# facebookresearch/Active-3D-Vision-and-Touch

Measured on AMD Instinct MI355X. Metric: mesh-recon iters/sec (fwd+bwd, 2562-vert GCN + 10k-pt Chamfer) at bs=64, higher is better.
Workload: dtype f32; 1 GPU; icosphere-4 template (2562 verts, 5120 faces), 3-stage GCN 20x300 cut 0.33, bs=64/GPU, 10000-pt Chamfer x3 draws, Adam, ellipsoid clouds (BASELINE.json configs[1]); global_batch=64, parallelism=dp1

## Files before the change

### active-3d-vision-and-touch_amd/csrc/capi.hip

```cpp
#include <stdarg.h>
#include <stdlib.h>
#include <string.h>

#include "../../include/a3vt.h"
#include <atomic>
#include <mutex>
#include <unordered_map>

#include "kernels.h"
#include "prims.h"

namespace a3vt {

static thread_local char g_err[512] = "";

void set_error(const char *fmt, ...) {
  va_list ap;
  va_start(ap, fmt);
  vsnprintf(g_err, sizeof(g_err), fmt, ap);
  va_end(ap);
}

__device__ float g_zero_page[64];
static const float *zero_page() {
// ... 178 lines not shown
  StackPlan p{};
  const size_t m = (size_t)batch * n_vert;
  p.x3 = mode == GEMM_FP32X3 && num_layers > 2 && rowgemm3_stack_ok((long long)m, hidden, mask_ld(hidden, cut_len));
  p.omode = mode == GEMM_BF16_OPERANDS ? GEMM_BF16_OPERANDS : GEMM_FP32;
  const bool split_ok = split_usable(split, n_vert, cut_len);
  p.quad = num_layers > 1 &&
           (rec >= 0 ? rec == 1 : use_csrq(batch, n_vert, hidden, cut_len, mode, split_ok ? csrq_max_degree() : max_degree));
  p.qsplit = p.quad && split_ok;
  p.qcols = p.quad ? kQuadCols : 0;
  p.rm_ld = hidden - p.qcols;
  p.rm_off = m * p.qcols;
  return p;
}

static int launch_stack_ell(const StackPlan &p, const a3vt_adj_split *split, const int32_t *rowptr, const int32_t *col,
                            const float *val, int n_vert, int32_t *ell, hipStream_t s) {
  if (p.qsplit) {
    const SplitRef r = split_ref(split);
    return launch_csrqs_image(r.rowptr, r.col, r.scale, r.cls, n_vert, ell, s);
  }
  return p.quad ? launch_csrq_ell(rowptr, col, val, n_vert, ell, s) : 0;
}

static StackLayout stack_layout(int batch, int n_vert, int in_features, int hidden, int num_layers, int cut_len,
                                int need_backward, int gemm_mode = 0) {
  StackLayout L{};
  const size_t m = (size_t)batch * n_vert;
  const int cpad = pad4(cut_len);
  Arena a;
  const int kmax = hidden > pad4(in_features) ? hidden : pad4(in_features);
  L.wt_stride = align_up((size_t)rowgemm_bt_rows(kmax) * pad16(kmax), 64);
  if (gemm_mode == GEMM_FP32X3 && L.wt_stride < 3 * (size_t)kX3ImageFloats) L.wt_stride = 3 * (size_t)kX3ImageFloats;
  L.wt = a.take(L.wt_stride * (num_layers > 1 ? num_layers - 1 : 1));
  L.ldza = cpad > 4 ? cpad : 4;
  L.za = a.take(m * L.ldza);
  L.z3 = a.take(2 * m * 4);
// ... 510 lines not shown
  if (int rc = hub_rows(rowptr, n_vert, max_degree, scratch + L.heavy, &heavy, s)) return rc;
  const StackPlan P = stack_plan(gemm_bf16, batch, n_vert, hidden, num_layers, cut_len, max_degree, split, -1);
  const int qcols = P.qcols, rm_ld = P.rm_ld;
  const size_t rm_off = P.rm_off;
  if (P.x3)
    if (int rc = launch_stack_images(GEMM_FP32X3, 1, weights, 1, num_layers - 1, in_features, hidden, ld_feats, hidden,
                                     scratch + L.wt, L.wt_stride, s))
      return rc;
  if (int rc = launch_stack_images(GEMM_FP32, 1, weights, 0, P.x3 ? 1 : num_layers - 1, in_features, hidden, ld_feats, hidden,
                                   scratch + L.wt, L.wt_stride, s))
    return rc;
  if (num_layers > 1) path_count(P.quad ? PATH_STACK_QUAD : PATH_STACK_ROWS);
  if (P.qsplit) path_count(PATH_STACK_SPLIT);
  if (num_layers > 1) stash_layout_record(masks, P.quad);
  int32_t *ell = reinterpret_cast<int32_t *>(scratch + L.ell);
  if (int rc = launch_stack_ell(P, split, rowptr, col, val, n_vert, ell, s)) return rc;
  const float *x = feats, *xq = nullptr;
  int ldx = ld_feats;
  for (int i = 0; i + 1 < num_layers; ++i) {
    const int k = i == 0 ? ld_feats : hidden;
    const bool l3 = P.x3 && i > 0;
    float *y = acts ? acts + S.act(i) : scratch + L.ping[i & 1];
    RowGemmArgs g{};
    g.a0 = g.a1 = x;
    g.lda0 = g.lda1 = ldx;
    g.ksplit = k;
    if (xq) {
      g.a0 = xq;
      g.ksplit = qcols;
      g.a0q_nvert = n_vert;
      g.a0q_quads = qcols / 4;
// ... 18 lines not shown
      g.zq_nvert = n_vert;
      g.zq_quads = cpad / 4;
      g.yq = y;
      g.yq_quads = qcols / 4;
      g.trash = scratch + L.z3;
    }
    {
      ProfScope ps(PROF_GEMM_FWD, s);
      if (int rc = launch_rowgemm(g, EPI_FWD_HIDDEN, s)) return rc;
    }
    if (P.quad) {
      uint8_t *sq = masks ? masks + S.signq(i) : nullptr;
      ProfScope psa(PROF_AGG, s);
      if (P.qsplit) {
        if (int rc = launch_csrqs_fwd(scratch + L.za, biases[i], cut_len, ell, n_vert, batch, y, qcols / 4, sq, 1, s)) return rc;
      } else if (int rc = launch_csrq_fwd(scratch + L.za, biases[i], cut_len, rowptr, col, val, heavy, ell, n_vert, batch, y, qcols / 4, sq, 1, s)) {
        return rc;
      }
      xq = y;
    } else if (cut_len > 0) {
      ProfScope psa(PROF_AGG, s);
      if (int rc = launch_csr_fwd(scratch + L.za, L.ldza, biases[i], cut_len, rowptr, col, val, heavy, n_vert, batch, y, hidden, mk, S.mld, 1, s))
        return rc;
    }
    x = y + rm_off - qcols;
    ldx = rm_ld;
  }
  const int klast = num_layers == 1 ? in_features : hidden;
  ProfScope pso(PROF_OUT, s);
  const SplitRef sref = split_ref(split);
  return launch_thin_fwd(x, ldx, klast, weights[num_layers - 1], biases[num_layers - 1], rowptr, col, val, heavy, n_vert,
// ... 50 lines not shown
  const StackLayout L = stack_layout(batch, n_vert, in_features, hidden, num_layers, cut_len, 1, gemm_bf16);
  const StackStash S = stack_stash(batch, n_vert, hidden, num_layers, cut_len, gemm_bf16);
  const size_t m = (size_t)batch * n_vert;
  const int cpad = pad4(cut_len);
  const int last = num_layers - 1;

  const SplitRef sref = split_ref(split);
  int32_t *heavyT;
  if (int rc = hub_rows(rowptrT, n_vert, max_degreeT, scratch + L.heavy, &heavyT, s)) return rc;
  const StackPlan P = stack_plan(gemm_bf16, batch, n_vert, hidden, num_layers, cut_len, max_degreeT, split,
                                 masks ? stash_layout_lookup(masks) : 0);
  const bool quad = P.quad;
  const int qcols = P.qcols, rm_ld = P.rm_ld;
  const size_t rm_off = P.rm_off;
  int32_t *ellT = reinterpret_cast<int32_t *>(scratch + L.ell);
  if (int rc = launch_stack_ell(P, split, rowptrT, colT, valT, n_vert, ellT, s)) return rc;
  {
    const float *xl = num_layers == 1 ? feats : acts + S.act(last - 1);
    const float *x = xl + rm_off - qcols;
    const int ldx = num_layers == 1 ? ld_feats : rm_ld;
    const int k = num_layers == 1 ? in_features : hidden;
    float *gprev = num_layers == 1 ? grad_feats : scratch + L.ping[0];
    const int ldg = num_layers == 1 ? ld_feats : hidden;
    ProfScope pso(PROF_OUT, s);
    if (int rc = launch_thin_bwd(x, ldx, k, weights[last], rowptrT, colT, valT, heavyT, n_vert, batch, grad_update,
                                 scratch + L.z3, num_layers > 1, gprev, ldg, ldg, scratch + L.thin_dw_slab,
                                 scratch + L.thin_db_slab, quad ? scratch + L.gq : nullptr, cpad / 4, quad ? xl : nullptr,
                                 qcols / 4, s, split ? &sref : nullptr))
      return rc;
    if (int rc = reduce_output_grads(scratch + L.thin_dw_slab, scratch + L.thin_db_slab, k, grad_weights[last], grad_biases[last],
                                     acc, s))
// ... 14 lines not shown
    float *g = scratch + L.ping[cur];
    float *dza = scratch + L.za;
    const float *xl = i == 0 ? feats : acts + S.act(i - 1);
    const bool xhyb = quad && i > 0;
    const float *x = xhyb ? xl + rm_off - qcols : xl;
    const int ldx = i == 0 ? ld_feats : (xhyb ? rm_ld : hidden);
    const int kin = i == 0 ? in_features : hidden;

    if (cut_len > 0 && quad) {
      const uint8_t *sq = masks + S.signq(i);
      ProfScope psa(PROF_AGG, s);
      if (P.qsplit) {
        if (int rc = launch_csrqs_bwd(scratch + L.gq, cut_len, ellT, n_vert, batch, dza, sq,
                                      scratch + L.db_slab + (size_t)i * L.db_layer_stride, s))
          return rc;
      } else if (int rc = launch_csrq_bwd(scratch + L.gq, cut_len, rowptrT, colT, valT, heavyT, ellT, n_vert, batch, dza, sq,
                                          scratch + L.db_slab + (size_t)i * L.db_layer_stride, s)) {
        return rc;
      }
    } else if (cut_len > 0) {
      ProfScope psa(PROF_AGG, s);
      if (int rc = launch_csr_bwd(g, hidden, cut_len, rowptrT, colT, valT, heavyT, n_vert, batch, dza, L.ldza,
                                  scratch + L.db_slab + (size_t)i * L.db_layer_stride, s))
        return rc;
    } else if (!acc) {
      if (int rc = launch_fill_zero(grad_biases[i], hidden, s)) return rc;
    }

    DwArgs d{};
    if (xhyb) {
      d.ldx_src = rm_ld;
// ... 809 lines not shown

int a3vt_dbg_path_counts(long long *counts, int n, int reset) {
  A3VT_CHECK_ARG(n >= 0 && (counts != nullptr || n == 0));
  for (int i = 0; i < n; ++i) counts[i] = i < PATH_COUNT ? g_path_counts[i].load(std::memory_order_relaxed) : 0;
  if (reset)
    for (auto &c : g_path_counts) c.store(0, std::memory_order_relaxed);
  return PATH_COUNT;
}

int a3vt_dbg_csr_algo(int algo) {
  A3VT_CHECK_ARG(algo >= 0 && algo <= 2);
  g_csr_algo = algo;
  return 0;
}

int a3vt_split3_bf16(const float *x, size_t n, uint16_t *hi, uint16_t *mid, uint16_t *lo, void *stream) {
  A3VT_CHECK_ARG(n == 0 || (x && hi && mid && lo));
  return launch_split3(x, n, hi, mid, lo, static_cast<hipStream_t>(stream));
}

int a3vt_check_finite(const float *data, size_t n, int32_t *flag, void *stream) {
  A3VT_CHECK_ARG(data && flag);
  return launch_check_finite(data, n, flag, static_cast<hipStream_t>(stream));
}

}
```

### active-3d-vision-and-touch_amd/csrc/gcn_csrq.hip

```cpp
#include "kernels.h"
#include "prims.h"

namespace a3vt {


constexpr int kCsrqThreads = 512;
constexpr int kHeavyDegQ = 64;
constexpr int kEllW = 8;

__global__ void csr_ell_build_kernel(const int32_t *__restrict__ rowptr, const int32_t *__restrict__ colidx,
                                     const float *__restrict__ val, int n_vert, i32x2 *__restrict__ ell,
                                     int32_t *__restrict__ degs) {
  const int v = blockIdx.x * blockDim.x + threadIdx.x;
  if (v >= n_vert) return;
  const int e0 = rowptr[v], n = rowptr[v + 1] - e0;
  degs[v] = n;
#pragma unroll
  for (int j = 0; j < kEllW; ++j)
    ell[(size_t)j * n_vert + v] = j < n ? i32x2{colidx[e0 + j], (int)f32_bits(val[e0 + j])} : i32x2{n_vert, 0};
}
size_t csrq_ell_ints(int n_vert) { return (size_t)n_vert * (2 * kEllW + 1) + 64; }
int launch_csrq_ell(const int32_t *rowptr, const int32_t *col, const float *val, int n_vert, int32_t *ell, hipStream_t s) {
  A3VT_LAUNCH(csr_ell_build_kernel, dim3(cdiv(n_vert, 256)), dim3(256), 0, s, rowptr, col, val, n_vert,
              reinterpret_cast<i32x2 *>(ell), ell + (size_t)n_vert * 2 * kEllW);
  A3VT_CHECK_LAUNCH();
  return 0;
}

template <int MODE, int VPT>
__global__ __launch_bounds__(kCsrqThreads) void csrq_kernel(const float *__restrict__ srcq, int nq, int parts,
                                                            const float *__restrict__ bias, int c,
                                                            const int32_t *__restrict__ rowptr,
                                                            const int32_t *__restrict__ colidx,
                                                            const float *__restrict__ val, int n_vert, int batch,
                                                            float *__restrict__ dst, int nq_dst,
                                                            uint8_t *__restrict__ signq, int relu, int heavy_thresh,
                                                            float *__restrict__ db_slab,
                                                            const int32_t *__restrict__ ellbuf) {
  extern __shared__ __attribute__((aligned(16))) float lds_raw[];
  __shared__ float red[2][kCsrqThreads / 64][4];
  const i32x2 *ell = reinterpret_cast<const i32x2 *>(ellbuf);
  const int32_t *degs = ellbuf + (size_t)n_vert * 2 * kEllW;
  f32x4 *tile0 = reinterpret_cast<f32x4 *>(lds_raw);
  const int xcd = blockIdx.x & 7, loc = blockIdx.x >> 3;
  const int jm = loc / parts, part = loc - jm * parts;
  const int b = xcd + 8 * jm;
  if (b >= batch) return;
  const int q_lo = part * nq / parts, q_hi = (part + 1) * nq / parts;
  if (q_lo >= q_hi) return;

  int vv[VPT], dg[VPT];
  bool on[VPT];
  int cj[VPT][kEllW];
  float wj[VPT][kEllW];
#pragma unroll
  for (int k = 0; k < VPT; ++k) {
    const int v = threadIdx.x + k * kCsrqThreads;
    on[k] = v < n_vert;
    vv[k] = on[k] ? v : n_vert - 1;
    dg[k] = degs[vv[k]];
#pragma unroll
    for (int j = 0; j < kEllW; ++j) {
      const i32x2 e = ell[(size_t)j * n_vert + vv[k]];
      const int e0 = e[0], e1 = e[1];
      cj[k][j] = e0;
      wj[k][j] = bits_f32((unsigned)e1);
    }
  }

  auto fetch = [&](int q, int k, f32x4 &v4, unsigned &bits) {
    const size_t plane = ((size_t)b * nq + q) * n_vert;
    v4 = reinterpret_cast<const f32x4 *>(srcq)[plane + vv[k]];
    bits = MODE == 1 ? signq[plane + vv[k]] : 0u;
  };
  auto park = [&](f32x4 *tile, int q, int k, f32x4 v4, unsigned bits) {
    if (MODE == 1) {
#pragma unroll
      for (int t = 0; t < 4; ++t) v4[t] = ((bits >> t) & 1u) ? v4[t] : 0.f;
    }
    (void)q;
    tile[vv[k]] = v4;
  };

  if (threadIdx.x < 2) tile0[(size_t)threadIdx.x * (n_vert + 1) + n_vert] = f32x4{0.f, 0.f, 0.f, 0.f};
  {
    f32x4 v4[VPT];
    unsigned bits[VPT];
#pragma unroll
    for (int k = 0; k < VPT; ++k) fetch(q_lo, k, v4[k], bits[k]);
#pragma unroll
    for (int k = 0; k < VPT; ++k) park(tile0, q_lo, k, v4[k], bits[k]);
  }
  __syncthreads();

  for (int q = q_lo; q < q_hi; ++q) {
    const int par = (q - q_lo) & 1;
    const f32x4 *tile = tile0 + (size_t)par * (n_vert + 1);
    f32x4 *tnext = tile0 + (size_t)(par ^ 1) * (n_vert + 1);
    const int ch = q * 4;
    const size_t plane = ((size_t)b * nq + q) * n_vert;
    const int qn = q + 1 < q_hi ? q + 1 : q;
    f32x4 nv4[VPT];
    unsigned nbits[VPT];
#pragma unroll
    for (int k = 0; k < VPT; ++k) fetch(qn, k, nv4[k], nbits[k]);
    f32x4 bs = {0.f, 0.f, 0.f, 0.f};
    if (MODE == 0) {
#pragma unroll
      for (int t = 0; t < 4; ++t)
        if (ch + t < c) bs[t] = bias[ch + t];
    }
    f32x4 bsum = {0.f, 0.f, 0.f, 0.f};
#pragma unroll
    for (int k = 0; k < VPT; ++k) {
      __builtin_amdgcn_sched_barrier(0);
      const int v = vv[k];
      const f32x4 own = tile[v];
      if (MODE == 1) {
#pragma unroll
        for (int t = 0; t < 4; ++t) bsum[t] += on[k] ? own[t] : 0.f;
      }
      f32x4 acc = {0.f, 0.f, 0.f, 0.f};
#pragma unroll
      for (int j = 0; j < kEllW; ++j) {
        {
          const f32x4 r = tile[cj[k][j]];
          const float w = wj[k][j];
          acc[0] = __builtin_fmaf(w, r[0], acc[0]);
          acc[1] = __builtin_fmaf(w, r[1], acc[1]);
          acc[2] = __builtin_fmaf(w, r[2], acc[2]);
          acc[3] = __builtin_fmaf(w, r[3], acc[3]);
        }
      }
      if (dg[k] > kEllW && dg[k] <= heavy_thresh) {
        const int ea = rowptr[v];
        for (int e = ea + kEllW; e < ea + dg[k]; ++e) {
          const f32x4 r = tile[colidx[e]];
          const float w = val[e];
#pragma unroll
          for (int t = 0; t < 4; ++t) acc[t] = __builtin_fmaf(w, r[t], acc[t]);
        }
      }
      if (!on[k] || dg[k] > heavy_thresh) continue;
      f32x4 o;
      if (MODE == 0) {
        unsigned bits = 0;
#pragma unroll
        for (int t = 0; t < 4; ++t) {
          const float pre = ch + t < c ? acc[t] + bs[t] : own[t];
          o[t] = (pre > 0.f || !relu) ? pre : 0.f;
          bits |= (pre > 0.f ? 1u : 0u) << t;
// ... 2 lines not shown
      } else {
#pragma unroll
        for (int t = 0; t < 4; ++t) o[t] = ch + t < c ? acc[t] : own[t];
      }
      *reinterpret_cast<f32x4 *>(dst + ((((size_t)b * nq_dst + q) * n_vert) + v) * 4) = o;
    }
    __builtin_amdgcn_sched_barrier(0);
    if (MODE == 1) {
#pragma unroll
      for (int t = 0; t < 4; ++t) bsum[t] = wave_sum(bsum[t]);
      if ((threadIdx.x & 63) == 0) {
#pragma unroll
        for (int t = 0; t < 4; ++t) red[par][threadIdx.x >> 6][t] = bsum[t];
      }
    }
    if (q + 1 < q_hi) {
#pragma unroll
      for (int k = 0; k < VPT; ++k) park(tnext, q + 1, k, nv4[k], nbits[k]);
    }
    __syncthreads();
    if (MODE == 1 && threadIdx.x < 4) {
      float sacc = 0.f;
#pragma unroll
      for (int w = 0; w < kCsrqThreads / 64; ++w) sacc += red[par][w][threadIdx.x];
      db_slab[(size_t)b * (nq * 4) + ch + threadIdx.x] = sacc;
    }
  }
}

template <int MODE>
__global__ __launch_bounds__(256) void csrq_heavy_kernel(const float *__restrict__ srcq, int nq,
                                                         const float *__restrict__ bias, int c,
                                                         const int32_t *__restrict__ rowptr,
                                                         const int32_t *__restrict__ colidx,
                                                         const float *__restrict__ val, int n_vert, int batch,
                                                         const int32_t *__restrict__ heavy, float *__restrict__ dst,
                                                         int nq_dst, uint8_t *__restrict__ signq, int relu) {
  __shared__ f32x4 red[8][32];
  const int hl = threadIdx.x & 31, sub = threadIdx.x >> 5;
  const int count = heavy[0];
  const bool on = hl < nq;
// ... 41 lines not shown
        const unsigned bits = signq[plane + v];
#pragma unroll
        for (int t = 0; t < 4; ++t) {
          own[t] = ((bits >> t) & 1u) ? own[t] : 0.f;
          o[t] = ch + t < c ? a[t] : own[t];
        }
      }
      *reinterpret_cast<f32x4 *>(dst + ((((size_t)b * nq_dst + hl) * n_vert) + v) * 4) = o;
    }
    __syncthreads();
  }
}

int csrq_max_degree() { return kEllW; }
bool csrq_fits(int n_vert, int cut_len) {
  return cut_len > 0 && pad4(cut_len) <= 128 && n_vert <= 6 * kCsrqThreads && ((size_t)n_vert + 1) * 32 <= 158 * 1024;
}

template <int MODE, int VPT>
static int launch_csrq_vpt(const float *srcq, int nq, const float *bias, int c, const int32_t *rowptr, const int32_t *col,
                           const float *val, const int32_t *heavy, const int32_t *ell, int n_vert, int batch, float *dst,
                           int nq_dst, uint8_t *signq, int relu, float *db_slab, hipStream_t s) {
  const size_t shmem = ((size_t)n_vert + 1) * 32;
  static OncePerDevice once;
  once.run([] {
    (void)hipFuncSetAttribute((const void *)csrq_kernel<MODE, VPT>, hipFuncAttributeMaxDynamicSharedMemorySize, 158 * 1024);
  });
  int parts = 256 / (((batch + 7) / 8) * 8);
  parts = parts < 1 ? 1 : parts > nq ? nq : parts;
  const int grid = 8 * ((batch + 7) / 8) * parts;
  A3VT_LAUNCH((csrq_kernel<MODE, VPT>), dim3(grid), dim3(kCsrqThreads), shmem, s, srcq, nq, parts, bias, c, rowptr, col, val,
              n_vert, batch, dst, nq_dst, signq, relu, heavy ? kHeavyDegQ : 0x7fffffff, db_slab, ell);
  A3VT_CHECK_LAUNCH();
  return 0;
}

template <int MODE>
static int launch_csrq(const float *srcq, const float *bias, int c, const int32_t *rowptr, const int32_t *col,
                       const float *val, const int32_t *heavy, const int32_t *ell, int n_vert, int batch, float *dst,
                       int nq_dst, uint8_t *signq, int relu, float *db_slab, hipStream_t s) {
  const int nq = pad4(c) / 4;
  if (!csrq_fits(n_vert, c) || nq_dst < nq || (MODE == 1 && (!signq || !db_slab))) {
    set_error("csrq: n_vert=%d c=%d output planes=%d unsupported", n_vert, c, nq_dst);
    return -1;
  }
  int rc;
  if (n_vert <= 4 * kCsrqThreads)
    rc = launch_csrq_vpt<MODE, 4>(srcq, nq, bias, c, rowptr, col, val, heavy, ell, n_vert, batch, dst, nq_dst, signq, relu, db_slab, s);
  else
    rc = launch_csrq_vpt<MODE, 6>(srcq, nq, bias, c, rowptr, col, val, heavy, ell, n_vert, batch, dst, nq_dst, signq, relu, db_slab, s);
  if (rc) return rc;
  if (heavy) {
    A3VT_LAUNCH(csrq_heavy_kernel<MODE>, dim3(2048), dim3(256), 0, s, srcq, nq, bias, c, rowptr, col, val, n_vert, batch,
                heavy, dst, nq_dst, signq, relu);
    A3VT_CHECK_LAUNCH();
  }
  return 0;
}

int launch_csrq_fwd(const float *zq, const float *bias, int c, const int32_t *rowptr, const int32_t *col,
                    const float *val, const int32_t *heavy, const int32_t *ell, int n_vert, int batch, float *yq,
                    int yq_quads, uint8_t *signq, int relu, hipStream_t s) {
  return launch_csrq<0>(zq, bias, c, rowptr, col, val, heavy, ell, n_vert, batch, yq, yq_quads, signq, relu, nullptr, s);
}
int launch_csrq_bwd(const float *gq, int c, const int32_t *rowptrT, const int32_t *colT, const float *valT,
                    const int32_t *heavyT, const int32_t *ellT, int n_vert, int batch, float *dzaq,
                    const uint8_t *signq, float *db_slab, hipStream_t s) {
  return launch_csrq<1>(gq, nullptr, c, rowptrT, colT, valT, heavyT, ellT, n_vert, batch, dzaq, pad4(c) / 4,
                        const_cast<uint8_t *>(signq), 0, db_slab, s);
}

}
```

### active-3d-vision-and-touch_amd/csrc/kernels.h

```cpp
#pragma once
#include <hip/hip_runtime.h>
#include <stddef.h>
#include <stdint.h>

namespace a3vt {

enum { EPI_PLAIN = 0, EPI_FWD_HIDDEN = 1, EPI_DX_MASK = 2 };
enum GemmMode { GEMM_FP32 = 0, GEMM_BF16_OPERANDS = 1, GEMM_BF16_STORAGE = 2, GEMM_FP32X3 = 3 };

struct RowGemmArgs {
  const float *a0;
  const float *a1;
  const float *bt;
  const float *zeros;
  uint8_t *maskb;
  float *c;
  float *c2;
  int lda0, lda1, ksplit, ldb;
  int bt_rows;
  int col0;
  int m, k, n_store;
  int ldc, ldc2, csplit, mld, moff;
  int no_relu;
  int plain_relu;
// ... 71 lines not shown

int launch_csr_fwd(const float *za, int ldza, const float *bias, int c, const int32_t *rowptr, const int32_t *col,
                   const float *val, const int32_t *heavy, int n_vert, int batch, float *y, int ldy, uint8_t *maskb,
                   int mld, int relu, hipStream_t s);
size_t csr_heavy_scratch_ints(int n_vert);
int csr_heavy_degree();
int launch_csr_heavy_list(const int32_t *rowptr, int n_vert, int32_t *heavy, hipStream_t s);
int launch_relu_split(const float *gy, int ldgy, const float *y, int ldy, int relu, int n_out, int cpad, int npad,
                      long long m, float *ga, float *dz, hipStream_t s);
int csr_bwd_num_slabs(int batch, int n_vert);
int launch_csr_bwd(const float *g, int ldg, int c, const int32_t *rowptrT, const int32_t *colT, const float *valT,
                   const int32_t *heavyT, int n_vert, int batch, float *dza, int lddza, float *db_slab, hipStream_t s);

bool csrq_fits(int n_vert, int cut_len);
int csrq_max_degree();
size_t csrq_ell_ints(int n_vert);
int launch_csrq_ell(const int32_t *rowptr, const int32_t *col, const float *val, int n_vert, int32_t *ell, hipStream_t s);
int launch_csrq_fwd(const float *zq, const float *bias, int c, const int32_t *rowptr, const int32_t *col,
                    const float *val, const int32_t *heavy, const int32_t *ell, int n_vert, int batch, float *yq,
                    int yq_quads ,
                    uint8_t *signq, int relu, hipStream_t s);
int launch_csrq_bwd(const float *gq, int c, const int32_t *rowptrT, const int32_t *colT, const float *valT,
                    const int32_t *heavyT, const int32_t *ellT, int n_vert, int batch, float *dzaq, const uint8_t *signq,
                    float *db_slab, hipStream_t s);
struct SplitRef {
  const int32_t *rowptr, *col;
  const float *scale;
  const uint8_t *cls;
};
bool csrqs_fits(int n_vert, int cut_len);
int csrqs_max_degree();
int launch_csrqs_image(const int32_t *rowptr, const int32_t *col, const float *scale, const uint8_t *cls, int n_vert,
                       int32_t *img, hipStream_t s);
int launch_csrqs_fwd(const float *zq, const float *bias, int c, const int32_t *img, int n_vert, int batch, float *yq,
                     int yq_quads, uint8_t *signq, int relu, hipStream_t s);
int launch_csrqs_bwd(const float *gq, int c, const int32_t *img, int n_vert, int batch, float *dzaq, const uint8_t *signq,
                     float *db_slab, hipStream_t s);
bool rowgemm_quad_major_ok(int m, int n_store, int cpad);

// ... 194 lines not shown
```

### active-3d-vision-and-touch_amd/lib.py

```python
import ctypes
import os
import subprocess

_HERE = os.path.dirname(os.path.abspath(__file__))
CSRC = os.path.join(_HERE, "csrc")
LIB_PATH = os.environ.get("A3VT_LIB", os.path.join(_HERE, "liba3vt.so"))
SOURCES = ["capi.hip", "gcn_gemm.hip", "gcn_gemmw.hip", "gcn_dww.hip", "gcn_gemm16.hip", "gcn_gemm3.hip", "gcn_csr.hip", "gcn_csrq.hip", "gcn_csrqs.hip", "gcn_bf16s.hip", "posenc.hip", "posenc_wide.hip", "bias_grad.hip", "bnrelu.hip", "conv5.hip", "conv5f.hip", "adam.hip", "sample.hip", "chamfer.hip", "nn_prune.hip",
           "pooling.hip", "fold.hip", "ddqn.hip", "qnet_input.hip", "latent_nn.hip"]
EXTRA_FLAGS = {"chamfer.hip": ["-fno-slp-vectorize"], "nn_prune.hip": ["-fno-slp-vectorize"],
               "gcn_csrq.hip": ["-fno-slp-vectorize"], "gcn_csrqs.hip": ["-fno-slp-vectorize"],
               "gcn_gemmw.hip": ["-std=c++20"], "gcn_dww.hip": ["-std=c++20"]}

_vp, _i, _sz, _u64 = ctypes.c_void_p, ctypes.c_int, ctypes.c_size_t, ctypes.c_uint64


class AdjSplit(ctypes.Structure):
    _fields_ = [("rowptr", _vp), ("col", _vp), ("scale", _vp), ("cls", _vp),
                ("max_degree", ctypes.c_int32), ("n_seam", ctypes.c_int32), ("n_centre", ctypes.c_int32)]


SIGNATURES = {
    "a3vt_version": (_i, []),
    "a3vt_last_error": (ctypes.c_char_p, []),
    "a3vt_csr_validate": (_i, [_vp, _vp, _i, _i]),
# ... 67 lines not shown
    "a3vt_fold_fwd": (_i, [_vp, _vp, _i, _vp, _vp, _vp, _vp, _vp, _i, _i, _i, _vp, _vp, _sz, _vp]),
    "a3vt_fold_bwd": (_i, [_vp, _vp, _i, _vp, _vp, _vp, _vp, _vp, _i, _i, _i, _vp, _vp, _vp, _vp, _vp, _vp, _vp, _vp, _sz, _vp]),
    "a3vt_ddqn_td": (_i, [_vp, _vp, _vp, _vp, _vp, _vp, _vp, _i, _i, _i, ctypes.c_float, _vp, _vp, _vp, _vp, _vp]),
    "a3vt_ddqn_td_bwd": (_i, [_vp, _vp, _vp, _i, _i, _vp, _vp]),
    "a3vt_latent_nearest_scratch_bytes": (_sz, [_i, _i, _i]),
    "a3vt_latent_nearest": (_i, [_vp, _vp, _i, _i, _vp, _vp, _i, _i, _i, _vp, _vp, _vp, _vp, _vp, _vp]),
    "a3vt_latent_nn_tile": (_i, []),
    "a3vt_latent_nn_query_floats": (_i, []),
    "a3vt_latent_nn_cached_rows": (_i, []),
    "a3vt_qnet_input_scratch_bytes": (_sz, [_i, _i, _i, _i, _i]),
    "a3vt_qnet_input_fwd": (_i, [_vp, _vp, _vp, _vp, _vp, _vp, _vp, _vp, _vp, _i, _i, _vp, _vp, _vp, _i, _i, _i, _vp, _i, _vp, _vp]),
    "a3vt_qnet_input_bwd": (_i, [_vp, _vp, _vp, _vp, _vp, _vp, _i, _i, _vp, _vp, _vp, _i, _i, _i, _vp, _i, _vp, _i,
                                 _vp, _vp, _vp, _vp, _vp, _vp, _vp, _vp, _vp, _vp]),
    "a3vt_dbg_csr_algo": (_i, [_i]),
    "a3vt_dbg_path_counts": (_i, [_vp, _i, _i]),
    "a3vt_dbg_nn_work": (_i, [_i, _vp]),
    "a3vt_split3_bf16": (_i, [_vp, _sz, _vp, _vp, _vp, _vp]),
    "a3vt_check_finite": (_i, [_vp, _sz, _vp, _vp]),
    "a3vt_profile_enable": (_i, [_i]),
    "a3vt_profile_read": (_i, [_vp, _vp]),
    "a3vt_profile_read_classes": (_i, [_vp, _vp, _i]),
}

_LIB = None


def build(force=False, verbose=False):
    return _build(force, verbose, LIB_PATH, os.path.join(_HERE, "build"))


# ... 58 lines not shown
```

### include/a3vt.h

```cpp
#ifndef A3VT_H
#define A3VT_H
#include <stddef.h>
#include <stdint.h>

#ifdef __cplusplus
extern "C" {
#endif

#define A3VT_VERSION 163

int a3vt_version(void);
const char *a3vt_last_error(void);

int a3vt_csr_validate(const int32_t *rowptr_host, const int32_t *col_host, int n_vert, int nnz);

size_t a3vt_gcn_stack_scratch_bytes(int batch, int n_vert, int in_features, int hidden, int num_layers,
                                    int cut_len, int need_backward);
size_t a3vt_gcn_stack_mask_bytes(int batch, int n_vert, int hidden, int num_layers, int cut_len);
size_t a3vt_gcn_stack_scratch_bytes_mode(int batch, int n_vert, int in_features, int hidden, int num_layers,
                                         int cut_len, int need_backward, int gemm_bf16);
int a3vt_gcn_stack_stash_bytes(int batch, int n_vert, int hidden, int num_layers, int cut_len, int gemm_bf16,
                               size_t *acts_bytes, size_t *mask_bytes);

int a3vt_gcn_stack_fwd(const float *feats, int ld_feats, int in_features,
// ... 159 lines not shown
                     float *dist_xy, int32_t *idx_xy, float *dist_yx, int32_t *idx_yx, float *cd,
                     void *scratch, void *stream);
size_t a3vt_chamfer_workspace_bytes(int draws, int batch, int p, int q);
int a3vt_chamfer_fwd_ws(const float *x, const float *y, int draws, int batch, int p, int q,
                        float *dist_xy, int32_t *idx_xy, float *dist_yx, int32_t *idx_yx, float *cd,
                        void *workspace, size_t workspace_bytes, int algo, void *stream);
int a3vt_chamfer_fwd_shared(const float *x, const float *y, int draws, int batch, int y_batch, int p, int q,
                            float *dist_xy, int32_t *idx_xy, float *dist_yx, int32_t *idx_yx, float *cd,
                            void *workspace, size_t workspace_bytes, int algo, void *stream);
int a3vt_chamfer_bwd(const float *x, const float *y, int draws, int batch, int p, int q,
                     const int32_t *idx_xy, const int32_t *idx_yx, const float *grad_cd,
                     float *grad_x, float *grad_y, void *stream);

int a3vt_dbg_csr_algo(int algo);

int a3vt_dbg_path_counts(long long *counts, int n, int reset);

int a3vt_dbg_nn_work(int enable, unsigned long long *out8);

int a3vt_split3_bf16(const float *x, size_t n, uint16_t *hi, uint16_t *mid, uint16_t *lo, void *stream);

size_t a3vt_fold_workspace_bytes(int batch, int points, int backward);
int a3vt_fold_fwd(const float *bias_s, const float *g, int k, const float *w1g, const float *w2, const float *b2, const float *w3,
                  const float *b3, int batch, int points, int width, float *y, void *workspace, size_t workspace_bytes, void *stream);
int a3vt_fold_bwd(const float *bias_s, const float *g, int k, const float *w1g, const float *w2, const float *b2, const float *w3,
                  const float *dy, int batch, int points, int width, float *d_bias_s, float *dg, float *dw1g, float *dw2, float *db2,
                  float *dw3, float *db3, void *workspace, size_t workspace_bytes, void *stream);

int a3vt_ddqn_td(const float *q_cur, const float *q_next_online, const float *q_next_target, const float *mask, const float *actions,
                 const float *rewards, const float *denom, int batch, int num_actions, int budget, float gamma, float *loss,
// ... 33 lines not shown
```

Before: 21.84 iters/s.

## Compact CSRQ ELL image, triple-buffer quad planes, and balance leftover quads

The ELL index image is rebuilt with separate weight and packed 16-bit byte-offset column planes, and its width is sized to the actual max degree (6–8). The CSRQ aggregation kernel now keeps a three-slot LDS ring with inline-asm loads and explicit vmcnt waits, so the next two quad planes are prefetched while the current one is gathered. Leftover quads that do not divide evenly across parts are split by vertex groups among all parts. This aims to cut register pressure and index traffic and to hide global load latency. In exchange it uses 1.5x more LDS per block, depends on hand-written waitcnt bookkeeping, and restricts n_vert so byte offsets fit in 16 bits.

```diff
diff --git a/active-3d-vision-and-touch_amd/csrc/capi.hip b/active-3d-vision-and-touch_amd/csrc/capi.hip
--- a/active-3d-vision-and-touch_amd/csrc/capi.hip
+++ b/active-3d-vision-and-touch_amd/csrc/capi.hip
@@ -216,12 +216,12 @@
 }
 
 static int launch_stack_ell(const StackPlan &p, const a3vt_adj_split *split, const int32_t *rowptr, const int32_t *col,
-                            const float *val, int n_vert, int32_t *ell, hipStream_t s) {
+                            const float *val, int n_vert, int slots, int32_t *ell, hipStream_t s) {
   if (p.qsplit) {
     const SplitRef r = split_ref(split);
     return launch_csrqs_image(r.rowptr, r.col, r.scale, r.cls, n_vert, ell, s);
   }
-  return p.quad ? launch_csrq_ell(rowptr, col, val, n_vert, ell, s) : 0;
+  return p.quad ? launch_csrq_ell(rowptr, col, val, n_vert, slots, ell, s) : 0;
 }
 
 static StackLayout stack_layout(int batch, int n_vert, int in_features, int hidden, int num_layers, int cut_len,
@@ -762,7 +762,8 @@
   if (P.qsplit) path_count(PATH_STACK_SPLIT);
   if (num_layers > 1) stash_layout_record(masks, P.quad);
   int32_t *ell = reinterpret_cast<int32_t *>(scratch + L.ell);
-  if (int rc = launch_stack_ell(P, split, rowptr, col, val, n_vert, ell, s)) return rc;
+  const int slots = csrq_slots(max_degree);
+  if (int rc = launch_stack_ell(P, split, rowptr, col, val, n_vert, slots, ell, s)) return rc;
   const float *x = feats, *xq = nullptr;
   int ldx = ld_feats;
   for (int i = 0; i + 1 < num_layers; ++i) {
@@ -811,7 +812,7 @@
       ProfScope psa(PROF_AGG, s);
       if (P.qsplit) {
         if (int rc = launch_csrqs_fwd(scratch + L.za, biases[i], cut_len, ell, n_vert, batch, y, qcols / 4, sq, 1, s)) return rc;
-      } else if (int rc = launch_csrq_fwd(scratch + L.za, biases[i], cut_len, rowptr, col, val, heavy, ell, n_vert, batch, y, qcols / 4, sq, 1, s)) {
+      } else if (int rc = launch_csrq_fwd(scratch + L.za, biases[i], cut_len, rowptr, col, val, heavy, ell, slots, n_vert, batch, y, qcols / 4, sq, 1, s)) {
         return rc;
       }
       xq = y;
@@ -892,7 +893,8 @@
   const int qcols = P.qcols, rm_ld = P.rm_ld;
   const size_t rm_off = P.rm_off;
   int32_t *ellT = reinterpret_cast<int32_t *>(scratch + L.ell);
-  if (int rc = launch_stack_ell(P, split, rowptrT, colT, valT, n_vert, ellT, s)) return rc;
+  const int slots = csrq_slots(max_degreeT);
+  if (int rc = launch_stack_ell(P, split, rowptrT, colT, valT, n_vert, slots, ellT, s)) return rc;
   {
     const float *xl = num_layers == 1 ? feats : acts + S.act(last - 1);
     const float *x = xl + rm_off - qcols;
@@ -937,7 +939,7 @@
         if (int rc = launch_csrqs_bwd(scratch + L.gq, cut_len, ellT, n_vert, batch, dza, sq,
                                       scratch + L.db_slab + (size_t)i * L.db_layer_stride, s))
           return rc;
-      } else if (int rc = launch_csrq_bwd(scratch + L.gq, cut_len, rowptrT, colT, valT, heavyT, ellT, n_vert, batch, dza, sq,
+      } else if (int rc = launch_csrq_bwd(scratch + L.gq, cut_len, rowptrT, colT, valT, heavyT, ellT, slots, n_vert, batch, dza, sq,
                                           scratch + L.db_slab + (size_t)i * L.db_layer_stride, s)) {
         return rc;
       }
@@ -1777,6 +1779,19 @@
   return 0;
 }
 
+int a3vt_dbg_csrq_image(int n_vert, int max_degree, long long *out6) {
+  A3VT_CHECK_ARG(n_vert > 0 && out6 != nullptr);
+  const int slots = csrq_slots(max_degree);
+  const CsrqImage im = csrq_image(n_vert, slots);
+  out6[0] = slots;
+  out6[1] = (long long)im.wgt;
+  out6[2] = (long long)im.cols;
+  out6[3] = (long long)im.degs;
+  out6[4] = (long long)im.ints;
+  out6[5] = (long long)csrq_ell_ints(n_vert);
+  return 0;
+}
+
 int a3vt_split3_bf16(const float *x, size_t n, uint16_t *hi, uint16_t *mid, uint16_t *lo, void *stream) {
   A3VT_CHECK_ARG(n == 0 || (x && hi && mid && lo));
   return launch_split3(x, n, hi, mid, lo, static_cast<hipStream_t>(stream));
diff --git a/active-3d-vision-and-touch_amd/csrc/gcn_csrq.hip b/active-3d-vision-and-touch_amd/csrc/gcn_csrq.hip
--- a/active-3d-vision-and-touch_amd/csrc/gcn_csrq.hip
+++ b/active-3d-vision-and-touch_amd/csrc/gcn_csrq.hip
@@ -7,28 +7,57 @@
 constexpr int kCsrqThreads = 512;
 constexpr int kHeavyDegQ = 64;
 constexpr int kEllW = 8;
-
+constexpr int kEllMinW = 6;
+
+int csrq_slots(int max_degree) {
+  return max_degree <= 0 || max_degree > kEllW ? kEllW : max_degree < kEllMinW ? kEllMinW : max_degree;
+}
+size_t csrq_ell_ints(int n_vert) { return csrq_image(n_vert, kEllW).ints + 64; }
 __global__ void csr_ell_build_kernel(const int32_t *__restrict__ rowptr, const int32_t *__restrict__ colidx,
-                                     const float *__restrict__ val, int n_vert, i32x2 *__restrict__ ell,
-                                     int32_t *__restrict__ degs) {
+                                     const float *__restrict__ val, int n_vert, int slots, int32_t *__restrict__ ell) {
   const int v = blockIdx.x * blockDim.x + threadIdx.x;
   if (v >= n_vert) return;
+  const CsrqImage im = csrq_image(n_vert, slots);
   const int e0 = rowptr[v], n = rowptr[v + 1] - e0;
-  degs[v] = n;
-#pragma unroll
-  for (int j = 0; j < kEllW; ++j)
-    ell[(size_t)j * n_vert + v] = j < n ? i32x2{colidx[e0 + j], (int)f32_bits(val[e0 + j])} : i32x2{n_vert, 0};
-}
-size_t csrq_ell_ints(int n_vert) { return (size_t)n_vert * (2 * kEllW + 1) + 64; }
-int launch_csrq_ell(const int32_t *rowptr, const int32_t *col, const float *val, int n_vert, int32_t *ell, hipStream_t s) {
-  A3VT_LAUNCH(csr_ell_build_kernel, dim3(cdiv(n_vert, 256)), dim3(256), 0, s, rowptr, col, val, n_vert,
-              reinterpret_cast<i32x2 *>(ell), ell + (size_t)n_vert * 2 * kEllW);
+  ell[im.degs + v] = n;
+  for (int j = 0; j < slots; ++j) ell[im.wgt + (size_t)j * n_vert + v] = j < n ? (int)f32_bits(val[e0 + j]) : 0;
+  for (int jp = 0; jp < (slots + 1) / 2; ++jp) {
+    const unsigned lo = 16u * (unsigned)(2 * jp < n ? colidx[e0 + 2 * jp] : n_vert);
+    const unsigned hi = 16u * (unsigned)(2 * jp + 1 < n && 2 * jp + 1 < slots ? colidx[e0 + 2 * jp + 1] : n_vert);
+    ell[im.cols + (size_t)jp * n_vert + v] = (int)(lo | (hi << 16));
+  }
+}
+int launch_csrq_ell(const int32_t *rowptr, const int32_t *col, const float *val, int n_vert, int slots, int32_t *ell,
+                    hipStream_t s) {
+  if (slots < kEllMinW || slots > kEllW || n_vert > 6 * kCsrqThreads) {
+    set_error("csrq index image: n_vert=%d slots=%d unsupported", n_vert, slots);
+    return -1;
+  }
+  A3VT_LAUNCH(csr_ell_build_kernel, dim3(cdiv(n_vert, 256)), dim3(256), 0, s, rowptr, col, val, n_vert, slots, ell);
   A3VT_CHECK_LAUNCH();
   return 0;
 }
 
-template <int MODE, int VPT>
-__global__ __launch_bounds__(kCsrqThreads) void csrq_kernel(const float *__restrict__ srcq, int nq, int parts,
+__device__ __forceinline__ void load16_uncounted(f32x4 &d, const f32x4 *src) {
+  asm volatile("global_load_dwordx4 %0, %1, off\n\ts_nop 0" : "=v"(d) : "v"(src) : "memory");
+}
+__device__ __forceinline__ void load8_uncounted(unsigned &d, const uint8_t *src) {
+  asm volatile("global_load_ubyte %0, %1, off\n\ts_nop 0" : "=v"(d) : "v"(src) : "memory");
+}
+__device__ __forceinline__ void wait_younger(int n) {
+  switch (n) {
+#define A3VT_W(N) case N: wait_vmcnt<N>(); break;
+#define A3VT_W4(N) A3VT_W(N) A3VT_W(N + 1) A3VT_W(N + 2) A3VT_W(N + 3)
+    A3VT_W(1) A3VT_W(2) A3VT_W(3) A3VT_W4(4) A3VT_W4(8) A3VT_W4(12) A3VT_W4(16) A3VT_W4(20) A3VT_W4(24) A3VT_W4(28)
+    A3VT_W4(32) A3VT_W4(36)
+#undef A3VT_W4
+#undef A3VT_W
+    default: wait_vmcnt<0>(); break;
+  }
+}
+
+template <int MODE, int VPT, int W>
+__global__ __launch_bounds__(kCsrqThreads) void csrq_kernel(const float *__restrict__ srcq, int nq, int parts, int shared,
                                                             const float *__restrict__ bias, int c,
                                                             const int32_t *__restrict__ rowptr,
                                                             const int32_t *__restrict__ colidx,
@@ -39,39 +68,37 @@
                                                             const int32_t *__restrict__ ellbuf) {
   extern __shared__ __attribute__((aligned(16))) float lds_raw[];
   __shared__ float red[2][kCsrqThreads / 64][4];
-  const i32x2 *ell = reinterpret_cast<const i32x2 *>(ellbuf);
-  const int32_t *degs = ellbuf + (size_t)n_vert * 2 * kEllW;
+  const CsrqImage im = csrq_image(n_vert, W);
   f32x4 *tile0 = reinterpret_cast<f32x4 *>(lds_raw);
   const int xcd = blockIdx.x & 7, loc = blockIdx.x >> 3;
   const int jm = loc / parts, part = loc - jm * parts;
   const int b = xcd + 8 * jm;
   if (b >= batch) return;
-  const int q_lo = part * nq / parts, q_hi = (part + 1) * nq / parts;
-  if (q_lo >= q_hi) return;
-
-  int vv[VPT], dg[VPT];
-  bool on[VPT];
-  int cj[VPT][kEllW];
-  float wj[VPT][kEllW];
+  const int n_own = shared ? nq / parts : (part + 1) * nq / parts - part * nq / parts;
+  const int q_lo = shared ? part * n_own : part * nq / parts;
+  const int n_quads = n_own + shared;
+  if (n_quads <= 0) return;
+  auto quad_of = [&](int i) { return i < n_own ? q_lo + i : nq - shared + (i - n_own); };
+  const int n_groups = (n_vert + 63) >> 6;
+  const int g_lo = part * n_groups / parts, g_hi = (part + 1) * n_groups / parts;
+
+  const int wave0 = __builtin_amdgcn_readfirstlane((int)threadIdx.x) & ~63;
+  int vv[VPT];
+  bool on[VPT], live[VPT], mine[VPT];
 #pragma unroll
   for (int k = 0; k < VPT; ++k) {
     const int v = threadIdx.x + k * kCsrqThreads;
+    live[k] = wave0 + k * kCsrqThreads < n_vert;
+    mine[k] = (wave0 >> 6) + k * (kCsrqThreads / 64) >= g_lo && (wave0 >> 6) + k * (kCsrqThreads / 64) < g_hi;
     on[k] = v < n_vert;
     vv[k] = on[k] ? v : n_vert - 1;
-    dg[k] = degs[vv[k]];
-#pragma unroll
-    for (int j = 0; j < kEllW; ++j) {
-      const i32x2 e = ell[(size_t)j * n_vert + vv[k]];
-      const int e0 = e[0], e1 = e[1];
-      cj[k][j] = e0;
-      wj[k][j] = bits_f32((unsigned)e1);
-    }
   }
 
   auto fetch = [&](int q, int k, f32x4 &v4, unsigned &bits) {
     const size_t plane = ((size_t)b * nq + q) * n_vert;
-    v4 = reinterpret_cast<const f32x4 *>(srcq)[plane + vv[k]];
-    bits = MODE == 1 ? signq[plane + vv[k]] : 0u;
+    load16_uncounted(v4, reinterpret_cast<const f32x4 *>(srcq) + plane + vv[k]);
+    bits = 0u;
+    if (MODE == 1) load8_uncounted(bits, signq + plane + vv[k]);
   };
   auto park = [&](f32x4 *tile, int q, int k, f32x4 v4, unsigned bits) {
     if (MODE == 1) {
@@ -82,28 +109,77 @@
     tile[vv[k]] = v4;
   };
 
-  if (threadIdx.x < 2) tile0[(size_t)threadIdx.x * (n_vert + 1) + n_vert] = f32x4{0.f, 0.f, 0.f, 0.f};
-  {
-    f32x4 v4[VPT];
-    unsigned bits[VPT];
-#pragma unroll
-    for (int k = 0; k < VPT; ++k) fetch(q_lo, k, v4[k], bits[k]);
-#pragma unroll
-    for (int k = 0; k < VPT; ++k) park(tile0, q_lo, k, v4[k], bits[k]);
-  }
+  f32x4 va[VPT], vb[VPT];
+  unsigned ba[VPT], bb[VPT];
+#pragma unroll
+  for (int k = 0; k < VPT; ++k) {
+    vb[k] = f32x4{0.f, 0.f, 0.f, 0.f};
+    bb[k] = 0u;
+  }
+  auto fetch_all = [&](int q, f32x4(&v4)[VPT], unsigned(&bits)[VPT]) {
+#pragma unroll
+    for (int k = 0; k < VPT; ++k) fetch(q, k, v4[k], bits[k]);
+  };
+  auto settle = [&](int younger, f32x4(&v4)[VPT], unsigned(&bits)[VPT]) {
+    wait_younger(younger);
+#pragma unroll
+    for (int k = 0; k < VPT; ++k) asm volatile("" : "+v"(v4[k]), "+v"(bits[k]));
+    __builtin_amdgcn_sched_barrier(0);
+  };
+  auto park_all = [&](f32x4 *tile, int q, f32x4(&v4)[VPT], unsigned(&bits)[VPT]) {
+#pragma unroll
+    for (int k = 0; k < VPT; ++k) park(tile, q, k, v4[k], bits[k]);
+  };
+  fetch_all(quad_of(0), va, ba);
+  if (1 < n_quads) fetch_all(quad_of(1), vb, bb);
+
+  int dg[VPT];
+  unsigned cp[VPT][(W + 1) / 2];
+  float wj[VPT][W];
+#pragma unroll
+  for (int k = 0; k < VPT; ++k) {
+    dg[k] = 0;
+    if (!live[k]) continue;
+    dg[k] = ellbuf[im.degs + vv[k]];
+#pragma unroll
+    for (int j = 0; j < W; ++j) wj[k][j] = bits_f32((unsigned)ellbuf[im.wgt + (size_t)j * n_vert + vv[k]]);
+#pragma unroll
+    for (int jp = 0; jp < (W + 1) / 2; ++jp) cp[k][jp] = (unsigned)ellbuf[im.cols + (size_t)jp * n_vert + vv[k]];
+  }
+
+  __builtin_amdgcn_s_waitcnt(0x0f70);
+  settle(0, va, ba);
+  settle(0, vb, bb);
+  const int n_load = VPT * (MODE == 1 ? 2 : 1);
+  int n_store = 0, n_store_shared = 0;
+#pragma unroll
+  for (int k = 0; k < VPT; ++k) {
+    const int st = live[k] && __ballot(on[k] && dg[k] <= heavy_thresh) != 0 ? (MODE == 0 && signq ? 2 : 1) : 0;
+    n_store += st;
+    n_store_shared += mine[k] ? st : 0;
+  }
+  n_store = __builtin_amdgcn_readfirstlane(n_store);
+  n_store_shared = __builtin_amdgcn_readfirstlane(n_store_shared);
+  auto stores_of = [&](int i) { return i < 0 ? 0 : i < n_own ? n_store : n_store_shared; };
+  const int stride = n_vert + 1;
+  if (threadIdx.x < 3) tile0[(size_t)threadIdx.x * stride + n_vert] = f32x4{0.f, 0.f, 0.f, 0.f};
+  park_all(tile0, quad_of(0), va, ba);
+  if (2 < n_quads) fetch_all(quad_of(2), va, ba);
   __syncthreads();
 
-  for (int q = q_lo; q < q_hi; ++q) {
-    const int par = (q - q_lo) & 1;
-    const f32x4 *tile = tile0 + (size_t)par * (n_vert + 1);
-    f32x4 *tnext = tile0 + (size_t)(par ^ 1) * (n_vert + 1);
+  auto quad = [&](int i, f32x4(&v4)[VPT], unsigned(&bits)[VPT]) {
+    const int q = quad_of(i);
+    const bool whole = i < n_own;
+    const int par = i & 1;
+    const int slot = i % 3;
+    const f32x4 *tile = tile0 + (size_t)slot * stride;
+    if (i + 1 < n_quads) {
+      settle((i + 2 < n_quads ? n_load : 0) + stores_of(i - 1) + stores_of(i - 2), v4, bits);
+      park_all(tile0 + (size_t)(slot == 2 ? 0 : slot + 1) * stride, quad_of(i + 1), v4, bits);
+      if (i + 3 < n_quads) fetch_all(quad_of(i + 3), v4, bits);
+    }
+    const size_t plane = ((size_t)b * nq + q) * n_vert;
     const int ch = q * 4;
-    const size_t plane = ((size_t)b * nq + q) * n_vert;
-    const int qn = q + 1 < q_hi ? q + 1 : q;
-    f32x4 nv4[VPT];
-    unsigned nbits[VPT];
-#pragma unroll
-    for (int k = 0; k < VPT; ++k) fetch(qn, k, nv4[k], nbits[k]);
     f32x4 bs = {0.f, 0.f, 0.f, 0.f};
     if (MODE == 0) {
 #pragma unroll
@@ -114,17 +190,22 @@
 #pragma unroll
     for (int k = 0; k < VPT; ++k) {
       __builtin_amdgcn_sched_barrier(0);
+      if (!live[k]) continue;
+      const bool gathers = whole || mine[k];
+      if (!gathers && !(MODE == 1 && part == 0)) continue;
       const int v = vv[k];
       const f32x4 own = tile[v];
       if (MODE == 1) {
 #pragma unroll
         for (int t = 0; t < 4; ++t) bsum[t] += on[k] ? own[t] : 0.f;
       }
+      if (!gathers) continue;
       f32x4 acc = {0.f, 0.f, 0.f, 0.f};
 #pragma unroll
-      for (int j = 0; j < kEllW; ++j) {
+      for (int j = 0; j < W; ++j) {
         {
-          const f32x4 r = tile[cj[k][j]];
+          const unsigned off = j & 1 ? cp[k][j / 2] >> 16 : cp[k][j / 2] & 0xffffu;
+          const f32x4 r = *reinterpret_cast<const f32x4 *>(reinterpret_cast<const char *>(tile) + off);
           const float w = wj[k][j];
           acc[0] = __builtin_fmaf(w, r[0], acc[0]);
           acc[1] = __builtin_fmaf(w, r[1], acc[1]);
@@ -132,9 +213,9 @@
           acc[3] = __builtin_fmaf(w, r[3], acc[3]);
         }
       }
-      if (dg[k] > kEllW && dg[k] <= heavy_thresh) {
+      if (dg[k] > W && dg[k] <= heavy_thresh) {
         const int ea = rowptr[v];
-        for (int e = ea + kEllW; e < ea + dg[k]; ++e) {
+        for (int e = ea + W; e < ea + dg[k]; ++e) {
           const f32x4 r = tile[colidx[e]];
           const float w = val[e];
 #pragma unroll
@@ -167,17 +248,17 @@
         for (int t = 0; t < 4; ++t) red[par][threadIdx.x >> 6][t] = bsum[t];
       }
     }
-    if (q + 1 < q_hi) {
-#pragma unroll
-      for (int k = 0; k < VPT; ++k) park(tnext, q + 1, k, nv4[k], nbits[k]);
-    }
     __syncthreads();
-    if (MODE == 1 && threadIdx.x < 4) {
+    if (MODE == 1 && threadIdx.x < 4 && (whole || part == 0)) {
       float sacc = 0.f;
 #pragma unroll
       for (int w = 0; w < kCsrqThreads / 64; ++w) sacc += red[par][w][threadIdx.x];
       db_slab[(size_t)b * (nq * 4) + ch + threadIdx.x] = sacc;
     }
+  };
+  for (int i = 0; i < n_quads; i += 2) {
+    quad(i, vb, bb);
+    if (i + 1 < n_quads) quad(i + 1, va, ba);
   }
 }
 
@@ -249,41 +330,52 @@
 
 int csrq_max_degree() { return kEllW; }
 bool csrq_fits(int n_vert, int cut_len) {
-  return cut_len > 0 && pad4(cut_len) <= 128 && n_vert <= 6 * kCsrqThreads && ((size_t)n_vert + 1) * 32 <= 158 * 1024;
-}
-
-template <int MODE, int VPT>
+  return cut_len > 0 && pad4(cut_len) <= 128 && n_vert <= 6 * kCsrqThreads && ((size_t)n_vert + 1) * 48 <= 158 * 1024;
+}
+
+template <int MODE, int VPT, int W>
 static int launch_csrq_vpt(const float *srcq, int nq, const float *bias, int c, const int32_t *rowptr, const int32_t *col,
                            const float *val, const int32_t *heavy, const int32_t *ell, int n_vert, int batch, float *dst,
                            int nq_dst, uint8_t *signq, int relu, float *db_slab, hipStream_t s) {
-  const size_t shmem = ((size_t)n_vert + 1) * 32;
+  const size_t shmem = ((size_t)n_vert + 1) * 48;
   static OncePerDevice once;
   once.run([] {
-    (void)hipFuncSetAttribute((const void *)csrq_kernel<MODE, VPT>, hipFuncAttributeMaxDynamicSharedMemorySize, 158 * 1024);
+    (void)hipFuncSetAttribute((const void *)csrq_kernel<MODE, VPT, W>, hipFuncAttributeMaxDynamicSharedMemorySize, 158 * 1024);
   });
   int parts = 256 / (((batch + 7) / 8) * 8);
   parts = parts < 1 ? 1 : parts > nq ? nq : parts;
   const int grid = 8 * ((batch + 7) / 8) * parts;
-  A3VT_LAUNCH((csrq_kernel<MODE, VPT>), dim3(grid), dim3(kCsrqThreads), shmem, s, srcq, nq, parts, bias, c, rowptr, col, val,
-              n_vert, batch, dst, nq_dst, signq, relu, heavy ? kHeavyDegQ : 0x7fffffff, db_slab, ell);
+  const int left = nq % parts;
+  const int shared = 3 * left <= parts + 2 ? left : 0;
+  A3VT_LAUNCH((csrq_kernel<MODE, VPT, W>), dim3(grid), dim3(kCsrqThreads), shmem, s, srcq, nq, parts, shared, bias, c, rowptr, col,
+              val, n_vert, batch, dst, nq_dst, signq, relu, heavy ? kHeavyDegQ : 0x7fffffff, db_slab, ell);
   A3VT_CHECK_LAUNCH();
   return 0;
 }
 
 template <int MODE>
 static int launch_csrq(const float *srcq, const float *bias, int c, const int32_t *rowptr, const int32_t *col,
-                       const float *val, const int32_t *heavy, const int32_t *ell, int n_vert, int batch, float *dst,
-                       int nq_dst, uint8_t *signq, int relu, float *db_slab, hipStream_t s) {
+                       const float *val, const int32_t *heavy, const int32_t *ell, int slots, int n_vert, int batch,
+                       float *dst, int nq_dst, uint8_t *signq, int relu, float *db_slab, hipStream_t s) {
   const int nq = pad4(c) / 4;
-  if (!csrq_fits(n_vert, c) || nq_dst < nq || (MODE == 1 && (!signq || !db_slab))) {
-    set_error("csrq: n_vert=%d c=%d output planes=%d unsupported", n_vert, c, nq_dst);
+  if (!csrq_fits(n_vert, c) || nq_dst < nq || (MODE == 1 && (!signq || !db_slab)) || slots < kEllMinW || slots > kEllW) {
+    set_error("csrq: n_vert=%d c=%d output planes=%d slots=%d unsupported", n_vert, c, nq_dst, slots);
     return -1;
   }
   int rc;
-  if (n_vert <= 4 * kCsrqThreads)
-    rc = launch_csrq_vpt<MODE, 4>(srcq, nq, bias, c, rowptr, col, val, heavy, ell, n_vert, batch, dst, nq_dst, signq, relu, db_slab, s);
-  else
-    rc = launch_csrq_vpt<MODE, 6>(srcq, nq, bias, c, rowptr, col, val, heavy, ell, n_vert, batch, dst, nq_dst, signq, relu, db_slab, s);
+#define A3VT_CSRQ(VPT, W)                                                                                              \
+  rc = launch_csrq_vpt<MODE, VPT, W>(srcq, nq, bias, c, rowptr, col, val, heavy, ell, n_vert, batch, dst, nq_dst, signq, \
+                                     relu, db_slab, s)
+  if (n_vert <= 4 * kCsrqThreads) {
+    if (slots == 6) A3VT_CSRQ(4, 6);
+    else if (slots == 7) A3VT_CSRQ(4, 7);
+    else A3VT_CSRQ(4, 8);
+  } else {
+    if (slots == 6) A3VT_CSRQ(6, 6);
+    else if (slots == 7) A3VT_CSRQ(6, 7);
+    else A3VT_CSRQ(6, 8);
+  }
+#undef A3VT_CSRQ
   if (rc) return rc;
   if (heavy) {
     A3VT_LAUNCH(csrq_heavy_kernel<MODE>, dim3(2048), dim3(256), 0, s, srcq, nq, bias, c, rowptr, col, val, n_vert, batch,
@@ -294,14 +386,14 @@
 }
 
 int launch_csrq_fwd(const float *zq, const float *bias, int c, const int32_t *rowptr, const int32_t *col,
-                    const float *val, const int32_t *heavy, const int32_t *ell, int n_vert, int batch, float *yq,
+                    const float *val, const int32_t *heavy, const int32_t *ell, int slots, int n_vert, int batch, float *yq,
                     int yq_quads, uint8_t *signq, int relu, hipStream_t s) {
-  return launch_csrq<0>(zq, bias, c, rowptr, col, val, heavy, ell, n_vert, batch, yq, yq_quads, signq, relu, nullptr, s);
+  return launch_csrq<0>(zq, bias, c, rowptr, col, val, heavy, ell, slots, n_vert, batch, yq, yq_quads, signq, relu, nullptr, s);
 }
 int launch_csrq_bwd(const float *gq, int c, const int32_t *rowptrT, const int32_t *colT, const float *valT,
-                    const int32_t *heavyT, const int32_t *ellT, int n_vert, int batch, float *dzaq,
+                    const int32_t *heavyT, const int32_t *ellT, int slots, int n_vert, int batch, float *dzaq,
                     const uint8_t *signq, float *db_slab, hipStream_t s) {
-  return launch_csrq<1>(gq, nullptr, c, rowptrT, colT, valT, heavyT, ellT, n_vert, batch, dzaq, pad4(c) / 4,
+  return launch_csrq<1>(gq, nullptr, c, rowptrT, colT, valT, heavyT, ellT, slots, n_vert, batch, dzaq, pad4(c) / 4,
                         const_cast<uint8_t *>(signq), 0, db_slab, s);
 }
 
diff --git a/active-3d-vision-and-touch_amd/csrc/kernels.h b/active-3d-vision-and-touch_amd/csrc/kernels.h
--- a/active-3d-vision-and-touch_amd/csrc/kernels.h
+++ b/active-3d-vision-and-touch_amd/csrc/kernels.h
@@ -109,15 +109,28 @@
 
 bool csrq_fits(int n_vert, int cut_len);
 int csrq_max_degree();
+int csrq_slots(int max_degree);
+struct CsrqImage {
+  size_t wgt, cols, degs, ints;
+};
+__host__ __device__ inline CsrqImage csrq_image(int n_vert, int slots) {
+  CsrqImage im;
+  im.wgt = 0;
+  im.cols = (size_t)slots * n_vert;
+  im.degs = im.cols + (size_t)((slots + 1) / 2) * n_vert;
+  im.ints = im.degs + n_vert;
+  return im;
+}
 size_t csrq_ell_ints(int n_vert);
-int launch_csrq_ell(const int32_t *rowptr, const int32_t *col, const float *val, int n_vert, int32_t *ell, hipStream_t s);
+int launch_csrq_ell(const int32_t *rowptr, const int32_t *col, const float *val, int n_vert, int slots, int32_t *ell,
+                    hipStream_t s);
 int launch_csrq_fwd(const float *zq, const float *bias, int c, const int32_t *rowptr, const int32_t *col,
-                    const float *val, const int32_t *heavy, const int32_t *ell, int n_vert, int batch, float *yq,
+                    const float *val, const int32_t *heavy, const int32_t *ell, int slots, int n_vert, int batch, float *yq,
                     int yq_quads ,
                     uint8_t *signq, int relu, hipStream_t s);
 int launch_csrq_bwd(const float *gq, int c, const int32_t *rowptrT, const int32_t *colT, const float *valT,
-                    const int32_t *heavyT, const int32_t *ellT, int n_vert, int batch, float *dzaq, const uint8_t *signq,
-                    float *db_slab, hipStream_t s);
+                    const int32_t *heavyT, const int32_t *ellT, int slots, int n_vert, int batch, float *dzaq,
+                    const uint8_t *signq, float *db_slab, hipStream_t s);
 struct SplitRef {
   const int32_t *rowptr, *col;
   const float *scale;
diff --git a/active-3d-vision-and-touch_amd/lib.py b/active-3d-vision-and-touch_amd/lib.py
--- a/active-3d-vision-and-touch_amd/lib.py
+++ b/active-3d-vision-and-touch_amd/lib.py
@@ -105,6 +105,7 @@
                                  _vp, _vp, _vp, _vp, _vp, _vp, _vp, _vp, _vp, _vp]),
     "a3vt_dbg_csr_algo": (_i, [_i]),
     "a3vt_dbg_path_counts": (_i, [_vp, _i, _i]),
+    "a3vt_dbg_csrq_image": (_i, [_i, _i, _vp]),
     "a3vt_dbg_nn_work": (_i, [_i, _vp]),
     "a3vt_split3_bf16": (_i, [_vp, _sz, _vp, _vp, _vp, _vp]),
     "a3vt_check_finite": (_i, [_vp, _sz, _vp, _vp]),
diff --git a/include/a3vt.h b/include/a3vt.h
--- a/include/a3vt.h
+++ b/include/a3vt.h
@@ -197,6 +197,8 @@
 
 int a3vt_dbg_csr_algo(int algo);
 
+int a3vt_dbg_csrq_image(int n_vert, int max_degree, long long *out6);
+
 int a3vt_dbg_path_counts(long long *counts, int n, int reset);
 
 int a3vt_dbg_nn_work(int enable, unsigned long long *out8);
```

Result: no change. 21.99 iters/s, median of 6 (+0.7%).
